# AVianEco/Softspoken

Hardware: AMD Instinct MI355X
Metric: audio-seconds processed/sec (whole node), 16 kHz mono (higher is better)
Workload: dtype f16x2

## Files before the change

softspoken_amd/build.py:

```python
from __future__ import annotations

import os
import subprocess
import sys

HERE = os.path.dirname(os.path.abspath(__file__))
CSRC = os.path.join(HERE, "csrc")
OBJ = os.path.join(CSRC, "_obj")
LIB = os.path.join(HERE, "libsoftspoken_hip.so")
DEV_LIB = os.path.join(HERE, "libsoftspoken_hip_dev.so")
SOURCES = ["conv2.hip", "conv2_ups.hip", "conv4.hip", "conv4_ups.hip", "conv1s.hip", "conv9s.hip", "conv9a.hip", "frontend.hip", "heads.hip", "weights.hip", "engine.hip", "host.hip", "abi.hip", "stream.hip", "separate.hip"]
HEADERS = [os.path.join(CSRC, h) for h in ("kernels.h", "engine.h", "dsp.h", "mfma_util.h", "conv4_forms.h", "stream16.h", "net.h", "bands.h")] + [os.path.join(os.path.dirname(HERE), "include", "softspoken.h")]
FLAGS = ["-O3", "--offload-arch=gfx950", "-fPIC", "-std=c++17", "-Wno-unused-value"]
EXTRA_FLAGS = {"frontend.hip": ["-fno-slp-vectorize"], "conv4.hip": ["-fno-slp-vectorize"], "conv4_ups.hip": ["-fno-slp-vectorize"],
               "conv1s.hip": ["-fno-slp-vectorize"], "conv9s.hip": ["-fno-slp-vectorize"], "conv9a.hip": ["-fno-slp-vectorize"]}
DEV_SOURCES = ("conv2.hip", "conv2_ups.hip", "conv4.hip", "conv4_ups.hip", "conv1s.hip", "frontend.hip", "engine.hip", "weights.hip", "abi.hip", "separate.hip")
JITTER_LIB = DEV_LIB


def _hipcc():
    for cand in (os.environ.get("HIPCC"), "/opt/rocm/bin/hipcc"):
        if cand and os.path.exists(cand):
            return cand
    return "hipcc"


def _stale(target, deps):
    if not os.path.exists(target):
        return True
    t = os.path.getmtime(target)
    return any(os.path.getmtime(d) > t for d in deps)


def build(force: bool = False, verbose: bool = True, dev: bool = False, jitter: bool = False) -> str:
    dev = dev or jitter
    os.makedirs(OBJ, exist_ok=True)
    hipcc = _hipcc()
    objs, procs = [], []
# ... 28 lines not shown
```

softspoken_amd/csrc/engine.h:

```cpp
#pragma once
#include "../../include/softspoken.h"
#include "kernels.h"
#include "net.h"

#include <map>
#include <string>
#include <vector>

namespace ss {

inline size_t pcm_bytes_per_sample(int format) {
    switch (format) {
        case SS_PCM_U8: case SS_PCM_S8: return 1;
        case SS_PCM_S16: case SS_PCM_S16BE: return 2;
        case SS_PCM_S24: case SS_PCM_S24BE: return 3;
        case SS_PCM_F64: case SS_PCM_F64BE: return 8;
        default: return 4;
    }
}

int fail(ss_ctx* c, int code, const std::string& msg);
const char* thread_error();

#define HIPCHK(c, expr)                                                                                   \
// ... 7 lines not shown
static_assert(sizeof(BlobEntry) == 152, "blob entry layout");
struct Blob {
    std::map<std::string, BlobEntry> e;
    const char* base = nullptr;
    size_t size = 0;
    bool has(const std::string& k) const { return e.count(k) != 0; }
    const float* f32(const std::string& k, size_t count, std::string& err) const;
};
bool parse_blob(const void* p, size_t n, Blob& b, std::string& err);

enum Precision { kFp32 = 0, kBf16 = 1, kF16x2 = 2 };

struct ConvPlan {
    std::string name;
    void* d_w2 = nullptr; float* d_bias2 = nullptr; float* d_res_bias = nullptr; float* d_rank1 = nullptr;
    void* d_w3 = nullptr; void* d_proj = nullptr; float* d_bias3 = nullptr;
    void* d_w_ups = nullptr;
    bool s1_range_proven = false;
    void* d_w_s1 = nullptr;
    void* d_w_s16 = nullptr;
    void* d_proj_s16 = nullptr;
    void* d_w_a16 = nullptr; void* d_w_ups16 = nullptr;
    void* d_w_upsr = nullptr;
    void* d_w_ups32 = nullptr;
    int ups32_nt = 1;
    int Cout = 0, NT = 1, C0 = 0, C1 = 0, R0 = 0, R1 = 0, H = 0, W = 0;
};

struct BlockPlan { ConvPlan A, B; };

struct FileRec {
    int64_t off = 0;
    int64_t n = 0;
    int64_t n_padded = 0;
    double duration = 0;
    int64_t W = 0, win_base = 0;
    int64_t bin_off = 0; int n_bins = 0;
};

struct StreamSet;
struct SepState;

struct SepPlan {
    int N = 0, hop = 0;
    int64_t W = 0, n_bins = 0, windows_run = 0;
    std::vector<ss_separation_range> ranges;
// ... 183 lines not shown
```

softspoken_amd/csrc/engine.hip:

```cpp
#include "engine.h"

#include <algorithm>
#include <chrono>
#include <cmath>
#include <cstdio>
#include <cstdlib>
#include <cstring>

namespace ss {

static thread_local std::string g_err;

int fail(ss_ctx* c, int code, const std::string& msg) {
    g_err = msg;
    if (c) c->err = msg;
    return code;
}
const char* thread_error() { return g_err.c_str(); }

double now_ms() { return std::chrono::duration<double, std::milli>(std::chrono::steady_clock::now().time_since_epoch()).count(); }

static int stat_id(ss_ctx* c, const std::string& name) {
    for (size_t i = 0; i < c->stats.size(); ++i) if (c->stats[i].name == name) return (int)i;
    KStat k; k.name = name; c->stats.push_back(k);
// ... 45 lines not shown
    c->dbg_n = 0; c->dbg_ws = 0; c->dbg_written = 0;
    for (Workspace& w : c->ws) free_ws(w);
}

static hipError_t ws_malloc(ss_ctx* c, void** p, size_t bytes) {
    if (c->fail_alloc_after >= 0 && c->fail_alloc_after-- == 0) { *p = nullptr; return hipErrorOutOfMemory; }
    return hipMalloc(p, bytes);
}

static hipError_t alloc_ws(ss_ctx* c, int n, hipStream_t stream, Workspace& w, std::string& what) {
    const size_t es = c->prec == kFp32 ? 4 : 2;
    size_t total = 0;
    std::vector<size_t> offs;
    for (const ActInfo& t : kActs) {
        offs.push_back(total + kActHeader);
        total += kActHeader + (((size_t)n * t.H * t.W * t.C * es + 255) & ~(size_t)255);
    }
    const int planes = c->prec == kF16x2 ? 2 : 1;
    const size_t feat_b = (size_t)n * 128 * 256 * 4, flat_b = (size_t)n * 64 * 4 * 256 * 4;
    hipError_t e = ws_malloc(c, &w.arena, total * planes);
    if (e != hipSuccess) { what = "activation workspace (" + std::to_string(total * planes >> 20) + " MiB)"; free_ws(w); return e; }
    if ((e = ws_malloc(c, (void**)&w.feat, feat_b)) != hipSuccess || (e = ws_malloc(c, (void**)&w.flat, flat_b)) != hipSuccess) {
        what = "activation workspace"; free_ws(w); return e;
    }
    for (int pl = 0; pl < planes; ++pl)
        for (size_t off : offs) {
            e = hipMemsetAsync((char*)w.arena + pl * total + off - kActHeader, 0, kActHeader, stream);
            if (e != hipSuccess) { what = "hipMemsetAsync"; free_ws(w); return e; }
        }
    const bool planar = c->prec == kF16x2 && dev_env("SOFTSPOKEN_LAYOUT", kActChunkPlanar ? 1 : 0) != 0;
    for (int i = 0; i < kActCount; ++i) {
        const ActInfo& t = kActs[i];
        w.t[i].p = (char*)w.arena + offs[i];
        if (c->prec != kFp32) w.t[i].s = act_stride(t.H, t.W, t.C, planar && !t.frag_order);
    }
    w.lo_delta = planes == 2 ? (int64_t)total : 0;
    w.bytes = (int64_t)(total * planes + feat_b + flat_b);
    w.chunk = n;
    return hipSuccess;
}

int ensure_workspace(ss_ctx* c, int n) {
    if (n <= c->ws[0].chunk) return SS_OK;
    HIPCHK(c, hipStreamSynchronize(c->stream));
    if (c->lane_stream) HIPCHK(c, hipStreamSynchronize(c->lane_stream));
    free_workspace(c);
// ... 59 lines not shown

template <typename LaunchFn>
static int conv_launch(ss_ctx* c, hipStream_t stream, const char* variant, const std::string& layer, ConvArgs& a, double flops, double bytes,
                       double issued, bool stamped, LaunchFn&& launch) {
    StageStamps stamps;
    if (stamped) if (int rc = stamps.begin(c, stream, layer, a)) return rc;
    {
        ScopedLaunch sl(c, stream, std::string(variant) + "/" + layer, flops, bytes, issued);
        HIPCHK(c, launch(a));
    }
    return stamps.end(c, stream, layer, a.N);
}

enum Form {
    kNoForm,
    kConv2,
    kConv4,
    kConv4UpsPlain,
    kConv4UpsRing,
    kConv2Ups,
    kConv1Stream16,
    kConv1Stream32,
    kConv9aStream,
    kConv9Stream
};
struct Launch { Form form = kNoForm; ConvArgs a{}; };
struct BlockRun { bool proj = false; Launch A, B, B2; };

static int prec4(const ss_ctx* c) { return c->prec == kF16x2 ? 2 : 1; }
static int ups32_mtw(const ConvPlan& p) { return dev_env("SOFTSPOKEN_UPS32_MTW", 2) == 2 && p.ups32_nt < 3 ? 2 : 1; }

static void fill_args(const ss_ctx* c, const Workspace& ws, int bi, int n, bool with_spec, BlockRun& r) {
    const Block& k = kBlocks[bi];
    const BlockPlan& p = c->convs[bi];
    auto T = [&](Act t) { return t == kNoAct ? ActTensor() : ws.t[t]; };
    const ActTensor x0 = T(k.x0), x1 = T(k.x1), h = T(k.first_in_loader ? kNoAct : k.h), rr = T(k.r), y = T(k.y), pool = T(k.pool);
    ConvArgs& a = r.A.a; ConvArgs& b = r.B.a;
    a = b = ConvArgs{};
    a.N = b.N = n; a.H = b.H = k.H; a.W = b.W = k.W; a.Cout = b.Cout = k.cout; a.relu = b.relu = 1; a.store_out = b.store_out = 1;
    a.lo_delta = b.lo_delta = ws.lo_delta; a.range_flag = b.range_flag = c->d_range_flag; a.dbg = b.dbg = base_dbg();
    a.src0 = x0.p; a.s_src0 = x0.s; a.src1 = x1.p; a.s_src1 = x1.s; a.C0 = k.c0; a.C1 = k.c1; a.out = h.p; a.s_out = h.s; a.bias = p.A.d_bias2;
    b.src0 = h.p; b.s_src0 = h.s; b.C0 = k.cout; b.out = y.p; b.s_out = y.s; b.pool_out = pool.p; b.s_pool = pool.s; b.wpk = p.B.d_w2;
    if (r.proj) {
        a.wpk = p.A.d_w3; a.plain = 1;
        b.bias = p.B.d_bias3; b.proj_w = p.B.d_proj; b.xp0 = x0.p; b.s_xp0 = x0.s; b.xp1 = x1.p; b.s_xp1 = x1.s; b.C0x = k.c0; b.C1x = k.c1;
    } else {
        a.wpk = p.A.d_w2; a.res_out = rr.p; a.res_bias = p.A.d_res_bias;
        b.bias = p.B.d_bias2; b.res_in = rr.p; b.rank1_w = p.B.d_rank1;
    }
    if (k.first_in_loader) { b.first_w = c->d_first_w; b.first_b = c->d_first_b; b.rank1_src = ws.feat; }
    if (k.flat_in_b) { b.flat_w = r.proj ? nullptr : c->d_flat_frag; b.flat_w4 = c->d_flat_frag4; b.flat_part = ws.flat; b.store_out = with_spec ? 1 : 0; }
}

static bool choose_tile(const ss_ctx* c, const ConvPlan& p, Launch& l) {
    if (c->prec != kFp32 && dev_env("SOFTSPOKEN_CONV4", 1) && conv_v4_supports(l.a, p.NT, c->num_cus, prec4(c))) l.form = kConv4;
    else if (c->prec != kF16x2) l.form = kConv2;
    return l.form != kNoForm;
}

static bool choose_A(const ss_ctx* c, const ConvPlan& p, Launch& l) {
    Launch u = l;
    if (c->prec == kF16x2 && p.d_w_upsr) {
        u.form = kConv4UpsRing; u.a.wpk = p.d_w_upsr;
        if (conv_upsr_supports(u.a, c->num_cus)) { l = u; return true; }
    }
    if (c->prec == kFp32 && p.d_w_ups32 && l.a.src1) {
        u.form = kConv2Ups; u.a.wpk = p.d_w_ups32;
        if (conv_ups32_supports(u.a, p.ups32_nt, ups32_mtw(p), c->num_cus)) { l = u; return true; }
    }
    return choose_tile(c, p, l);
}

static bool choose_B(const ss_ctx* c, const Block& k, const ConvPlan& p, BlockRun& r) {
    if (c->prec == kF16x2 && k.first_in_loader && p.d_w_s16 && dev_env("SOFTSPOKEN_C1S", 1)) {
        Launch s = r.B;
        s.form = dev_env("SOFTSPOKEN_C1S_FORM", 16) == 32 && p.d_w_s1 ? kConv1Stream32 : kConv1Stream16;
        s.a.wpk = s.form == kConv1Stream16 ? p.d_w_s16 : p.d_w_s1;
        s.a.relu = 1 | (dev_env("SOFTSPOKEN_C1S_ABLATE", 0) << 4);
        s.a.plain = p.s1_range_proven && dev_env("SOFTSPOKEN_C1S_TRACK", 0) == 0;
        if (conv1_stream_supports(s.a)) {
            if (dev_env("SOFTSPOKEN_C1S", 1) == 2) { r.B2 = r.B; if (!choose_tile(c, p, r.B2)) return false; }
            r.B = s;
            return true;
        }
// ... 32 lines not shown
        fill_args(c, ws, bi, n, with_spec, r);
        if (choose_proj(c, k, p, r)) return true;
        r = BlockRun();
    }
    fill_args(c, ws, bi, n, with_spec, r);
    if (!k.first_in_loader && !choose_A(c, p.A, r.A)) return false;
    return choose_B(c, k, p.B, r);
}

static double launch_macs(const Block& k, bool isA, bool proj, int n) {
    const double px = (double)n * k.H * k.W, cin = k.c0 + k.c1;
    if (isA) return px * k.cout * (9.0 * cin + (proj ? 0.0 : cin));
    return px * k.cout * (9.0 * k.cout + (proj ? cin : 0.0) + (k.first_in_loader ? 1 : 0)) + (k.first_in_loader ? px * 32 * 9 : 0.0) +
           (k.flat_in_b ? px * 32 * 4 : 0.0);
}
static double launch_bytes(const Block& k, bool isA, bool proj, int n, double es, bool store_y) {
    const double px = (double)n * k.H * k.W, x = k.c0 + k.c1 / 4.0;
    if (isA) return px * es * (x + k.cout + (proj ? 0 : k.cout));
    return px * es * ((k.first_in_loader ? 4.0 / es : k.cout) + (proj ? x : k.r != kNoAct ? k.cout : 0) + (store_y ? k.cout : 0) + (k.pool != kNoAct ? k.cout / 4.0 : 0));
}
static double launch_issued(const Block& k, Form f, int n) {
    const double px = (double)n * k.H * k.W;
    switch (f) {
        case kConv4UpsRing: case kConv2Ups: return px * k.cout * (9.0 * k.c0 + 4.0 * k.c1 + (k.c0 + k.c1));
        case kConv4UpsPlain: return px * k.cout * (9.0 * k.c0 + 4.0 * k.c1);
        case kConv9aStream: return conv9a_stream_issued_macs(n);
        case kConv9Stream: return conv9_stream_issued_macs(n);
        default: return -1.0;
    }
}
static int flat_groups_of(const ss_ctx* c, Form f) {
    return f == kConv9Stream ? conv9_stream_flat_groups(dev_env("SOFTSPOKEN_C9S_ROWS", 32)) : f == kConv4 ? conv_v4_flat_groups() : conv_v2_flat_groups(c->bf16);
}

static int launch_form(ss_ctx* c, hipStream_t stream, const ConvPlan& p, Launch& l, double flops, double bytes, double issued) {
    const int cus = c->num_cus;
    auto go = [&](const char* variant, auto&& launch) { return conv_launch(c, stream, variant, p.name, l.a, flops, bytes, issued, l.form != kConv4UpsPlain, launch); };
    switch (l.form) {
        case kConv2: return go(conv_v2_variant(l.a, c->bf16, p.NT, cus), [&](ConvArgs& x) { return launch_conv3x3_v2(x, c->bf16, p.NT, cus, stream); });
        case kConv4: return go(conv_v4_variant(l.a, p.NT, cus, prec4(c)), [&](ConvArgs& x) { return launch_conv3x3_v4(x, p.NT, cus, prec4(c), stream); });
        case kConv4UpsPlain: return go(conv_ups_variant(), [&](ConvArgs& x) { return launch_conv3x3_ups(x, cus, stream); });
        case kConv4UpsRing: return go(conv_upsr_variant(), [&](ConvArgs& x) { return launch_conv3x3_upsr(x, cus, stream); });
        case kConv2Ups: return go(conv_ups32_variant(p.ups32_nt, ups32_mtw(p)), [&](ConvArgs& x) { return launch_conv3x3_ups32(x, p.ups32_nt, ups32_mtw(p), cus, stream); });
        case kConv1Stream16: case kConv1Stream32: {
            const int form = l.form == kConv1Stream16 ? 16 : 32;
            return go(conv1_stream_variant(l.a, form), [&](ConvArgs& x) { return launch_conv1_stream(x, form, dev_env("SOFTSPOKEN_C1S_ROWS", 32), cus, stream); });
        }
        case kConv9aStream:
            return go(conv9a_stream_variant(), [&](ConvArgs& x) { return launch_conv9a_stream(x, dev_env("SOFTSPOKEN_C9A_ROWS", 32), dev_env("SOFTSPOKEN_C9A_GRID", 0), cus, stream); });
        case kConv9Stream:
            return go(conv9_stream_variant(), [&](ConvArgs& x) { return launch_conv9_stream(x, dev_env("SOFTSPOKEN_C9S_ROWS", 32), dev_env("SOFTSPOKEN_C9S_GRID", 0), cus, stream); });
        case kNoForm: break;
    }
    return fail(c, SS_ERR_STATE, "no kernel form chosen for " + p.name);
}

static int run_block(ss_ctx* c, Workspace& ws, hipStream_t stream, int bi, int n, bool with_spec) {
    const Block& k = kBlocks[bi];
    const BlockPlan& p = c->convs[bi];
    BlockRun r;
    if (!choose_block(c, ws, bi, n, with_spec, r))
        return fail(c, SS_ERR_STATE, "f16x2: no kernel form for " + (k.first_in_loader || r.A.form != kNoForm ? p.B.name : p.A.name));
    const bool hasA = r.A.form != kNoForm, store_y = r.B.a.store_out != 0;
    for (Act t : {hasA ? k.h : kNoAct, hasA && !r.proj ? k.r : kNoAct, store_y ? k.y : kNoAct, k.pool})
        if (t != kNoAct) c->dbg_written |= (uint64_t)1 << t;
    const double es = c->prec == kBf16 ? 2 : 4;
    for (Launch* l : {&r.A, &r.B, &r.B2}) {
        if (l->form == kNoForm) continue;
        const bool isA = l == &r.A;
        if (int rc = launch_form(c, stream, isA ? p.A : p.B, *l, 2.0 * launch_macs(k, isA, r.proj, n), launch_bytes(k, isA, r.proj, n, es, store_y),
                                 launch_issued(k, l->form, n)))
            return rc;
// ... 354 lines not shown
```

softspoken_amd/csrc/kernels.h:

```cpp
#pragma once
#include <hip/hip_runtime.h>
#include <stdint.h>
#include <atomic>
#include <cstdlib>

namespace ss {

#ifdef SS_DEVBUILD
static inline int dev_env(const char* name, int dflt) { const char* v = getenv(name); return v ? atoi(v) : dflt; }
#else
static constexpr int dev_env(const char*, int dflt) { return dflt; }
#endif

inline hipError_t allow_full_lds(const void* kernel, std::atomic<uint64_t>& done) {
    int dev = 0;
    hipError_t e = hipGetDevice(&dev);
    if (e != hipSuccess) return e;
    const uint64_t bit = 1ull << (dev & 63);
    if (done.load(std::memory_order_acquire) & bit) return hipSuccess;
    e = hipFuncSetAttribute(kernel, hipFuncAttributeMaxDynamicSharedMemorySize, 160 * 1024);
    if (e == hipSuccess) done.fetch_or(bit, std::memory_order_release);
    return e;
}

// ... 102 lines not shown
hipError_t launch_conv3x3_ups32(const ConvArgs& a, int NT, int MTW, int num_cus, hipStream_t s);

bool conv1_stream_supports(const ConvArgs& a);
const char* conv1_stream_variant(const ConvArgs& a, int form);
size_t conv1_stream_weight_bytes();
hipError_t launch_conv1_stream(const ConvArgs& a, int form, int rows_per_unit, int num_cus, hipStream_t s);

bool conv9_stream_supports(const ConvArgs& a);
const char* conv9_stream_variant();
size_t conv9_stream_proj_bytes();
size_t conv9_stream_flat_bytes();
bool conv9_stream_rows_ok(int rows_per_unit);
int conv9_stream_flat_groups(int rows_per_unit);
double conv9_stream_issued_macs(int N);
hipError_t launch_conv9_stream(const ConvArgs& a, int rows_per_unit, int grid_override, int num_cus, hipStream_t s);

bool conv9a_stream_supports(const ConvArgs& a);
const char* conv9a_stream_variant();
size_t conv9a_stream_ups_bytes();
bool conv9a_stream_rows_ok(int rows_per_unit);
double conv9a_stream_issued_macs(int N);
hipError_t launch_conv9a_stream(const ConvArgs& a, int rows_per_unit, int grid_override, int num_cus, hipStream_t s);

struct Head1dWeights { float w1[4][4][3], b1[4], w2[4][4][3], wr[4][4], b2r[4], wo[4], bo, fscale; };
hipError_t launch_mask_head_parts(const float* parts, int n_parts, const float* flat_bias, const Head1dWeights& hw, float* logits,
                                  int N, hipStream_t s);
hipError_t launch_spec_tail(const void* x, int64_t lo_delta, const float* w , const float* bias, float* spec, int N, int prec,
                            hipStream_t s);

static constexpr int kMelLo = 10, kMelHi = 32, kMelPitch = 43;
struct FrontendTables {
    const float4* pretw;
    const float2* w2048;
    const int* mel_start;
    const int* mel_count;
    const int* mel_off;
    const float* mel_w;
    int mel_nw;
    const float* mel_wp;
    int dbg;
    const float2* win2;
    const float2* twt;
    const float2* wkt;
    const float* mel_wq;
    const int* mel_p0;
};
// ... 54 lines not shown
```

softspoken_amd/csrc/weights.hip:

```cpp
#include "engine.h"

#include <algorithm>
#include <cmath>
#include <cstring>

namespace ss {

const float* Blob::f32(const std::string& k, size_t count, std::string& err) const {
    auto it = e.find(k);
    if (it == e.end()) { err = "weights blob: missing tensor '" + k + "'"; return nullptr; }
    if (it->second.dtype != 0 || it->second.nbytes != count * 4) {
        err = "weights blob: tensor '" + k + "' has wrong dtype/size"; return nullptr;
    }
    return (const float*)(base + it->second.offset);
}

bool parse_blob(const void* p, size_t n, Blob& b, std::string& err) {
    if (n < 16 || memcmp(p, "SSWBLOB1", 8) != 0) { err = "weights blob: bad magic"; return false; }
    uint32_t cnt; memcpy(&cnt, (const char*)p + 8, 4);
    if (16 + (size_t)cnt * sizeof(BlobEntry) > n) { err = "weights blob: truncated table"; return false; }
    b.base = (const char*)p; b.size = n;
    for (uint32_t i = 0; i < cnt; ++i) {
        BlobEntry en; memcpy(&en, (const char*)p + 16 + (size_t)i * sizeof(BlobEntry), sizeof(BlobEntry));
        en.name[95] = 0;
// ... 207 lines not shown
}

static void pack_ups_stream16(const Folded& w3, int c0, std::vector<char>& out, bool& range_ok) {
    out.assign((size_t)2 * 2 * 4 * 2 * 2 * 1024, 0);
    static const int lo_of[2][2] = {{0, 1}, {0, 2}}, hi_of[2][2] = {{0, 2}, {1, 2}};
    for (int a = 0; a < 2; ++a)
        for (int ty = 0; ty < 2; ++ty)
            for (int f = 0; f < 4; ++f)
                for (int u = 0; u < 2; ++u)
                    for (int l = 0; l < 64; ++l)
                        for (int j = 0; j < 8; ++j) {
                            const int b = f >> 1, tx = f & 1, i = l & 15, co = 8 * (i >> 2) + 4 * u + (i & 3), ci = c0 + 8 * (l >> 4) + j;
                            double sum = 0.0;
                            for (int dy = lo_of[a][ty]; dy <= hi_of[a][ty]; ++dy)
                                for (int dx = lo_of[b][tx]; dx <= hi_of[b][tx]; ++dx) sum += (double)w3.w[((size_t)co * w3.cin + ci) * 9 + dy * 3 + dx];
                            const float v = (float)sum;
                            const uint16_t hi = f2h(v), lo = f2h(v - h2f(hi));
                            if ((hi & 0x7c00u) == 0x7c00u) range_ok = false;
                            const size_t off = ((size_t)((((a * 2 + ty) * 4 + f) * 2 + u) * 2) * 64 + l) * 16 + (size_t)j * 2;
                            memcpy(&out[off], &hi, 2); memcpy(&out[off + 1024], &lo, 2);
                        }
}

static void pack_conv_split_upsr(const Folded& w3, const Folded& wr, int c0, int c1, std::vector<char>& out, bool& range_ok) {
    const size_t ent_r = (size_t)10 * 2048, ent_rh = ent_r + 256, ent_u = (size_t)17 * 2048;
    const int nreg = c0 / 32, nups = c1 / 32, ngroups = w3.cout / 32;
    const size_t group = (size_t)nreg * (ent_rh + ent_r) + (size_t)nups * 2 * ent_u;
    out.assign((size_t)ngroups * group, 0);
    auto put = [&](size_t off_hi, size_t off_lo, float v) {
        const uint16_t hi = f2h(v), lo = f2h(v - h2f(hi));
        if ((hi & 0x7c00u) == 0x7c00u) range_ok = false;
        memcpy(&out[off_hi], &hi, 2); memcpy(&out[off_lo], &lo, 2);
    };
    static const int lo_of[2][2] = {{0, 1}, {0, 2}}, hi_of[2][2] = {{0, 2}, {1, 2}};
    for (int g = 0; g < ngroups; ++g) {
        const size_t gb = (size_t)g * group;
        for (int ci = 0; ci < nreg; ++ci) {
            const size_t eh = gb + (size_t)ci * (ent_rh + ent_r), el = eh + ent_rh;
            for (int t = 0; t < 10; ++t)
                for (int s = 0; s < 2; ++s)
                    for (int l = 0; l < 64; ++l)
                        for (int e = 0; e < 8; ++e) {
                            const int co = g * 32 + (l & 31), k = ci * 32 + s * 16 + (l >> 5) * 8 + e;
                            const float v = t < 9 ? w3.w[((size_t)co * w3.cin + k) * 9 + t] : wr.w[(size_t)co * wr.cin + k];
                            const size_t off = (size_t)t * 2048 + ((size_t)s * 64 + l) * 16 + (size_t)e * 2;
                            put(eh + off, el + off, v);
// ... 270 lines not shown
                bh[co] = q; worst = std::max(worst, q);
            }
            for (int co = 0; co < cout; ++co) {
                double q = std::fabs((double)b2r[co]) + std::fabs((double)fr.w[co]) * fmax;
                for (int ci = 0; ci < cout; ++ci)
                    for (int t = 0; t < 9; ++t) q += std::fabs((double)f2.w[((size_t)co * cout + ci) * 9 + t]) * bh[ci];
                worst = std::max(worst, q);
            }
            B.s1_range_proven = std::isfinite(worst) && worst < 60000.0;
        }
        out.B = B;
        return SS_OK;
    }
    const int NTA = (c->prec == kF16x2 && NT == 3) ? 1 : NT;
    ConvPlan A; A.name = name + ".A"; A.Cout = cout; A.NT = NTA; A.C0 = cin0; A.C1 = cin1; A.H = H; A.W = W;
    if ((rc = dev_upload(c, &A.d_bias2, f1.b.data(), cout * 4))) return rc;
    if (c->prec == kF16x2) pack_conv_split(f1, &fr, NTA, pk, c->split_range_ok); else pack_conv_v2(f1, &fr, c->bf16, NT, pk);
    if ((rc = dev_upload(c, (char**)&A.d_w2, pk.data(), pk.size()))) return rc;
    if ((rc = dev_upload(c, &A.d_res_bias, fr.b.data(), cout * 4))) return rc;
    if (c->prec == kF16x2 && NTA == 1 && cin0 >= 64 && cin0 % 32 == 0 && cin1 % 32 == 0 && (cin1 >= 32 || dev_env("SOFTSPOKEN_UPSR", 1) >= 2)) {
        pack_conv_split_upsr(f1, fr, cin0, cin1, pk, c->split_range_ok);
        if (pk.size() != conv_upsr_weight_bytes(cin0, cin1, cout)) return fail(c, SS_ERR_STATE, "pack_conv_split_upsr: size");
        if ((rc = dev_upload(c, (char**)&A.d_w_upsr, pk.data(), pk.size()))) return rc;
    }
    if (c->prec == kFp32 && cin1 >= 16 && cin0 % 16 == 0 && cin1 % 16 == 0 && cout % 32 == 0 && H % 16 == 0 && dev_env("SOFTSPOKEN_UPS32", 1)) {
        A.ups32_nt = dev_env("SOFTSPOKEN_UPS32_NT", 1);
        if (A.ups32_nt < 1 || A.ups32_nt > 3 || (cout / 32) % A.ups32_nt) A.ups32_nt = 1;
        pack_conv_v2_ups(f1, fr, cin0, cin1, A.ups32_nt, pk);
        if (pk.size() != conv_ups32_weight_bytes(cin0, cin1, cout)) return fail(c, SS_ERR_STATE, "pack_conv_v2_ups: size");
        if ((rc = dev_upload(c, (char**)&A.d_w_ups32, pk.data(), pk.size()))) return rc;
    }
    if (c->bf16) {
        pack_conv_v2(f1, nullptr, true, NT, pk);
        if ((rc = dev_upload(c, (char**)&A.d_w3, pk.data(), pk.size()))) return rc;
    }
    if (c->prec == kF16x2) {
        pack_conv_split(f1, nullptr, NTA, pk, c->split_range_ok);
        if ((rc = dev_upload(c, (char**)&A.d_w3, pk.data(), pk.size()))) return rc;
        if (cin1 >= 32 && cin0 >= 32 && cout == 32) {
            pack_conv_split_ups(f1, cin0, cin1, pk, c->split_range_ok);
            if (pk.size() != conv_ups_weight_bytes(cin0, cin1)) return fail(c, SS_ERR_STATE, "pack_conv_split_ups: size");
            if ((rc = dev_upload(c, (char**)&A.d_w_ups, pk.data(), pk.size()))) return rc;
            if (cin0 == 32 && cin1 == 32 && H == 128 && W == 256) {
                pack_conv_stream16(f1, pk, c->split_range_ok);
                if (pk.size() != conv1_stream_weight_bytes()) return fail(c, SS_ERR_STATE, "pack_conv_stream16: size");
                if ((rc = dev_upload(c, (char**)&A.d_w_a16, pk.data(), pk.size()))) return rc;
// ... 155 lines not shown
```

Measured before the change: 35390.

## Add streaming fused skip+upsample conv kernel for 64x128 decoder A-conv

Adds a new streaming kernel for the f16x2 decoder conv that fuses the 3x3 skip conv, the folded 2x upsample conv and the 1x1 residual projection. Each wave walks rows of a 32-wide strip, holding a register ring of weights staged through LDS and software-pipelining row loads against MFMA groups. The kernel is chosen by default for the 64x128, 64+64->32 layer ahead of the existing ups-ring kernel. It targets redundant activation reads and per-tile launch overhead. The cost is a specialised, shape-locked kernel with heavy register pressure. A debug workspace-poison option is also added.

```diff
diff --git a/softspoken_amd/build.py b/softspoken_amd/build.py
--- a/softspoken_amd/build.py
+++ b/softspoken_amd/build.py
@@ -9,11 +9,11 @@
 OBJ = os.path.join(CSRC, "_obj")
 LIB = os.path.join(HERE, "libsoftspoken_hip.so")
 DEV_LIB = os.path.join(HERE, "libsoftspoken_hip_dev.so")
-SOURCES = ["conv2.hip", "conv2_ups.hip", "conv4.hip", "conv4_ups.hip", "conv1s.hip", "conv9s.hip", "conv9a.hip", "frontend.hip", "heads.hip", "weights.hip", "engine.hip", "host.hip", "abi.hip", "stream.hip", "separate.hip"]
+SOURCES = ["conv2.hip", "conv2_ups.hip", "conv4.hip", "conv4_ups.hip", "conv1s.hip", "conv9s.hip", "conv9a.hip", "conv8a.hip", "frontend.hip", "heads.hip", "weights.hip", "engine.hip", "host.hip", "abi.hip", "stream.hip", "separate.hip"]
 HEADERS = [os.path.join(CSRC, h) for h in ("kernels.h", "engine.h", "dsp.h", "mfma_util.h", "conv4_forms.h", "stream16.h", "net.h", "bands.h")] + [os.path.join(os.path.dirname(HERE), "include", "softspoken.h")]
 FLAGS = ["-O3", "--offload-arch=gfx950", "-fPIC", "-std=c++17", "-Wno-unused-value"]
 EXTRA_FLAGS = {"frontend.hip": ["-fno-slp-vectorize"], "conv4.hip": ["-fno-slp-vectorize"], "conv4_ups.hip": ["-fno-slp-vectorize"],
-               "conv1s.hip": ["-fno-slp-vectorize"], "conv9s.hip": ["-fno-slp-vectorize"], "conv9a.hip": ["-fno-slp-vectorize"]}
+               "conv1s.hip": ["-fno-slp-vectorize"], "conv9s.hip": ["-fno-slp-vectorize"], "conv9a.hip": ["-fno-slp-vectorize"], "conv8a.hip": ["-fno-slp-vectorize"]}
 DEV_SOURCES = ("conv2.hip", "conv2_ups.hip", "conv4.hip", "conv4_ups.hip", "conv1s.hip", "frontend.hip", "engine.hip", "weights.hip", "abi.hip", "separate.hip")
 JITTER_LIB = DEV_LIB
 
diff --git a/softspoken_amd/csrc/conv8a.hip b/softspoken_amd/csrc/conv8a.hip
--- /dev/null
+++ b/softspoken_amd/csrc/conv8a.hip
@@ -0,0 +1,301 @@
+#include "kernels.h"
+#include "stream16.h"
+#include <algorithm>
+#include <type_traits>
+#include <utility>
+
+namespace ss {
+
+namespace {
+
+constexpr int kH8 = 64, kW8 = 128, kStrips8 = 4;
+constexpr uint32_t kRow2 = kW8 * 64, kRow7 = (kW8 / 2) * 64;
+constexpr uint32_t kChunk2 = kH8 * kRow2, kChunk7 = (kH8 / 2) * kRow7;
+constexpr int kSkip8 = 2 * 9 * 2048;
+constexpr int kUps8 = 2 * 4 * 4 * 2048;
+constexpr int kProj8 = 4 * 2048;
+constexpr int kTile8 = kSkip8 + kUps8 + kProj8;
+constexpr uint32_t kRWin = (kH8 / 2) * (kW8 / 16) * 2048;
+
+struct G8 { int kind, off, k, a, b, flags; };
+template <int DY, int RF, int PROJ, int C7FIRST>
+struct Seq8 {
+    G8 g[40];
+    int n;
+    constexpr void c2_groups() {
+        for (int k = 0; k < 2; ++k)
+            for (int dxi = 0; dxi < 3; ++dxi) {
+                bool first = true;
+                for (int dyi = 0; dyi < 3; ++dyi)
+                    if ((DY >> dyi) & 1) { g[n++] = G8{0, ((k * 9 + dyi * 3 + dxi) * 2) * 1024, k, dyi, dxi, (first ? 1 : 0) | (first && !RF && k == 1 && dxi == 0 ? 4 : 0)}; first = false; }
+                if (dxi == 1 && PROJ) g[n++] = G8{1, kSkip8 + kUps8 + k * 2048, k, 0, 0, 0};
+            }
+        if (RF && !C7FIRST) g[n - 1].flags |= 2;
+    }
+    constexpr void c7_groups() {
+        if (PROJ) g[n++] = G8{3, kSkip8 + kUps8 + 2 * 2048, 0, 0, 0, 0};
+        for (int k = 0; k < 2; ++k)
+            for (int pt = 0; pt < 2; ++pt) {
+                bool first = true;
+                for (int rf = 0; rf < 4; ++rf)
+                    if ((RF >> rf) & 1) { g[n++] = G8{2, kSkip8 + (((k * 4 + rf) * 4 + pt) * 2) * 1024, k, rf, pt, (first ? 1 : 0) | (first && k == 1 && pt == 1 ? 4 : 0)}; first = false; }
+            }
+    }
+    constexpr Seq8() : g{}, n(0) {
+        if (RF && C7FIRST) c7_groups();
+        c2_groups();
+        if (RF && !C7FIRST) c7_groups();
+    }
+};
+template <int DY, int RF, int PROJ, int STOREH, int EDGE, int INIT, int C7OFF, int LAST>
+struct SD8 {
+    static constexpr int dy = DY, rf = RF, proj = PROJ, storeh = STOREH, edge = EDGE, init = INIT, c7off = C7OFF, last = LAST;
+    static constexpr int c7first = C7OFF != 0;
+    static constexpr Seq8<DY, RF, PROJ, c7first> seq{};
+};
+using StepPro = SD8<1, 8, 0, 0, 1, 1, -1, 0>;
+using StepEvenFirst = SD8<3, 14, 1, 0, 0, 3, 0, 0>;
+using StepOdd = SD8<7, 0, 1, 1, 0, 0, 0, 0>;
+using StepEven = SD8<7, 15, 1, 1, 0, 3, 0, 0>;
+using StepEvenLast = SD8<7, 7, 1, 1, 0, 1, 0, 0>;
+using StepOddLast = SD8<6, 0, 1, 1, 0, 0, 0, 0>;
+using StepEpi = SD8<4, 1, 0, 1, 1, 0, 0, 1>;
+static_assert(StepPro::seq.n == 10 && StepEvenFirst::seq.n == 27 && StepOdd::seq.n == 20 && StepEven::seq.n == 37 && StepEvenLast::seq.n == 33 &&
+              StepOddLast::seq.n == 14 && StepEpi::seq.n == 10, "groups per step");
+static_assert((2 + 10) % 3 == 0 && (0 + 27) % 3 == 0 && (0 + 20) % 3 == 2 && (2 + 37) % 3 == 0 && (2 + 33) % 3 == 2 && (2 + 14) % 3 == 1 &&
+              (1 + 10) % 3 == 2, "ring phases");
+
+template <int... I, typename F>
+__device__ __forceinline__ void static_for_(std::integer_sequence<int, I...>, F&& f) { (f(std::integral_constant<int, I>{}), ...); }
+template <int N, typename F>
+__device__ __forceinline__ void static_for(F&& f) { static_for_(std::make_integer_sequence<int, N>{}, f); }
+
+struct C8Row7 { u32x4 f[2]; u32x4 h[2]; };
+struct C8Ring { u32x4 w[3][4]; };
+
+}
+
+__global__ __launch_bounds__(64 * kS1Waves) __attribute__((amdgpu_waves_per_eu(2, 2)))
+void conv3x3_upsr_stream16_kernel(ConvArgs a, int rows_per_unit, int total_units) {
+    extern __shared__ __attribute__((aligned(16))) char smem[];
+    const int tid = threadIdx.x, lane = tid & 63, wave = __builtin_amdgcn_readfirstlane(tid >> 6);
+    const int g = lane >> 4, c = lane & 15;
+    const int u = __builtin_amdgcn_readfirstlane(((int)blockIdx.x >> 3) & 1);
+    const int pair = __builtin_amdgcn_readfirstlane(((int)blockIdx.x & 7) + 8 * ((int)blockIdx.x >> 4)), npairs = (int)gridDim.x >> 1;
+    {
+        const char* src = (const char*)a.wpk + (size_t)u * kTile8;
+        for (int p = tid; p < kTile8 / 16; p += 64 * kS1Waves) *(u32x4*)(smem + p * 16) = *(const u32x4*)(src + (size_t)p * 16);
+    }
+    const f32x4 bias = *(const f32x4*)(a.bias + 16 * u + 4 * g), rbias = *(const f32x4*)(a.res_bias + 16 * u + 4 * g);
+    __syncthreads();
+
+    const char* fl = smem + lane * 16;
+    auto rsrc_of = [](const void* p, uint32_t bytes) { return __builtin_amdgcn_make_buffer_rsrc(const_cast<void*>(p), 0, (int)bytes, 0x00020000); };
+    auto ld16 = [](__amdgpu_buffer_rsrc_t rs, uint32_t vo, int so) { return __builtin_bit_cast(u32x4, __builtin_amdgcn_raw_buffer_load_b128(rs, (int)vo, so, 0)); };
+    const uint32_t px2 = a.s_src0.pix, ch2 = a.s_src0.chunk, px7 = a.s_src1.pix, ch7 = a.s_src1.chunk;
+    const uint32_t vpix = (uint32_t)(2 * c) * px2 + (uint32_t)g * 16u, vpix7 = (uint32_t)c * px7 + (uint32_t)g * 16u;
+    const uint32_t vout = (uint32_t)(2 * c) * 64u + 32u * (uint32_t)u + 8u * (uint32_t)g;
+    const uint32_t vr = (uint32_t)(c >> 3) * 2048u + (uint32_t)(32 * (g & 1) + 4 * (c & 7)) * 32u + 16u * (uint32_t)(g >> 1);
+    const int bands = kH8 / rows_per_unit;
+    const int64_t lo = a.lo_delta;
+    uint32_t ovf = 0;
+    C8Ring ring;
+    uint32_t far_ = 65536u;
+    asm volatile("" : "+v"(far_));
+    const char* fl_hi = fl + far_;
+    auto rd_group = [&](int slot, const G8 gd) {
+        const char* p = gd.off + (gd.kind >= 2 ? 4096 + 1024 : 1024) < 65536 ? fl + gd.off : fl_hi + (gd.off - 65536);
+        ring.w[slot][0] = *(const u32x4*)(p); ring.w[slot][1] = *(const u32x4*)(p + 1024);
+        if (gd.kind >= 2) {
+            const int d = gd.kind == 2 ? 4096 : 2048;
+            ring.w[slot][2] = *(const u32x4*)(p + d); ring.w[slot][3] = *(const u32x4*)(p + d + 1024);
+        }
+    };
+    { constexpr G8 g0 = StepPro::seq.g[0], g1 = StepPro::seq.g[1]; rd_group(2, g0); rd_group(0, g1); }
+
+    for (int unit = pair * kS1Waves + wave; unit < total_units; unit += npairs * kS1Waves) {
+        const int s = unit % kStrips8, b = (unit / kStrips8) % bands, n = unit / (kStrips8 * bands);
+        const int x0 = 32 * s, y0 = b * rows_per_unit, ylast = y0 + rows_per_unit - 1;
+        const uint32_t hpix = (uint32_t)(c < 8 ? max(x0 - 1, 0) : min(x0 + 32, kW8 - 1)) * px2 + (uint32_t)g * 16u;
+        const uint32_t hpix7 = (uint32_t)(c < 8 ? max(x0 / 2 - 1, 0) : min(x0 / 2 + 16, kW8 / 2 - 1)) * px7 + (uint32_t)g * 16u;
+        const uint32_t hkeep = (c < 8 ? s > 0 : s < kStrips8 - 1) ? 0xffffffffu : 0u;
+        const char* c2w = (const char*)a.src0 + (size_t)n * 2 * kChunk2;
+        const char* c7w = (const char*)a.src1 + (size_t)n * 2 * kChunk7;
+        const __amdgpu_buffer_rsrc_t rs2[2] = {rsrc_of(c2w, 2 * kChunk2), rsrc_of(c2w + lo, 2 * kChunk2)};
+        const __amdgpu_buffer_rsrc_t rs7[2] = {rsrc_of(c7w, 2 * kChunk7), rsrc_of(c7w + lo, 2 * kChunk7)};
+        char* ow = (char*)a.out + (size_t)n * kChunk2;
+        const __amdgpu_buffer_rsrc_t rso[2] = {rsrc_of(ow, kChunk2), rsrc_of(ow + lo, kChunk2)};
+        const __amdgpu_buffer_rsrc_t rsr = rsrc_of((char*)a.res_out + (size_t)u * lo + (size_t)n * kRWin, kRWin);
+
+        auto load_chunk = [&](S16RowH& H, int k, int r) {
+            const int so = (min(max(r, 0), kH8 - 1) * kW8 + x0) * (int)px2 + k * (int)ch2;
+#pragma unroll
+            for (int pq = 0; pq < 2; ++pq) {
+                H.f[0][pq] = ld16(rs2[pq], vpix, so);
+                H.f[1][pq] = ld16(rs2[pq], vpix, so + (int)px2);
+                H.h[pq] = ld16(rs2[pq], hpix, so - x0 * (int)px2);
+            }
+        };
+        auto load_row7 = [&](C8Row7 (&K)[2], int r7) {
+            const int so = (min(max(r7, 0), kH8 / 2 - 1) * (kW8 / 2) + x0 / 2) * (int)px7;
+#pragma unroll
+            for (int k = 0; k < 2; ++k)
+#pragma unroll
+                for (int pq = 0; pq < 2; ++pq) {
+                    K[k].f[pq] = ld16(rs7[pq], vpix7, so + k * (int)ch7);
+                    K[k].h[pq] = ld16(rs7[pq], hpix7, so - (x0 / 2) * (int)px7 + k * (int)ch7);
+                }
+        };
+        S16RowH Hrow[2][2];
+        C8Row7 K[2];
+        f32x4 A[4][2];
+        f32x4 R[2], RU, RUa, RUb;
+        uint32_t ovt = 0;
+
+        auto step = [&](auto cur, auto next, auto rho4_c, auto ph_c, int rho) {
+            using Cur = decltype(cur); using Next = decltype(next);
+            constexpr int RHO4 = decltype(rho4_c)::value, PH = decltype(ph_c)::value, N = Cur::seq.n;
+            S16RowH (&Hc)[2] = Hrow[RHO4 & 1];
+            const int Y = (rho + Cur::c7off) >> 1;
+            S16RowH (&Hn)[2] = Hrow[(RHO4 & 1) ^ 1];
+            if constexpr (!Cur::last && (Cur::rf == 0 || Cur::c7first)) load_chunk(Hn[0], 0, rho + 1);
+            if constexpr (Cur::rf != 0 && !Cur::c7first) load_row7(K, Y);
+            auto mask_row7 = [&]() {
+                const uint32_t rk = !Cur::edge || (unsigned)Y < (unsigned)(kH8 / 2) ? 0xffffffffu : 0u;
+#pragma unroll
+                for (int k = 0; k < 2; ++k)
+#pragma unroll
+                    for (int pq = 0; pq < 2; ++pq)
+#pragma unroll
+                        for (int e = 0; e < 4; ++e) {
+                            if constexpr (Cur::edge) K[k].f[pq][e] &= rk;
+                            K[k].h[pq][e] &= hkeep & rk;
+                        }
+            };
+            if constexpr (Cur::c7first) mask_row7();
+            {
+                const uint32_t rk = !Cur::edge || (unsigned)rho < (unsigned)kH8 ? 0xffffffffu : 0u;
+#pragma unroll
+                for (int k = 0; k < 2; ++k)
+#pragma unroll
+                    for (int pq = 0; pq < 2; ++pq)
+#pragma unroll
+                        for (int e = 0; e < 4; ++e) {
+                            if constexpr (Cur::edge) { Hc[k].f[0][pq][e] &= rk; Hc[k].f[1][pq][e] &= rk; }
+                            Hc[k].h[pq][e] &= hkeep & rk;
+                        }
+            }
+            if constexpr (Cur::init & 1) { A[(RHO4 + 1) & 3][0] = bias; A[(RHO4 + 1) & 3][1] = bias; }
+            if constexpr (Cur::init & 2) { A[(RHO4 + 2) & 3][0] = bias; A[(RHO4 + 2) & 3][1] = bias; }
+            u32x4 B[2][2];
+            static_for<N>([&](auto I) {
+                constexpr int i = decltype(I)::value, slot = (PH + i) % 3;
+                constexpr G8 gd = Cur::seq.g[i];
+                if constexpr (i + 2 < N) { constexpr G8 gn = Cur::seq.g[i + 2]; rd_group((PH + i + 2) % 3, gn); }
+                else { constexpr G8 gn = Next::seq.g[i + 2 - N]; rd_group((PH + i + 2) % 3, gn); }
+                if constexpr ((gd.flags & 4) != 0 && !Cur::last) load_chunk(Hn[1], 1, rho + 1);
+                if constexpr (gd.kind == 0 && (gd.flags & 1)) {
+#pragma unroll
+                    for (int pq = 0; pq < 2; ++pq) { B[0][pq] = s16_operand(Hc[gd.k], gd.b - 1, 0, pq); B[1][pq] = s16_operand(Hc[gd.k], gd.b - 1, 1, pq); }
+                }
+                if constexpr (gd.kind == 2 && (gd.flags & 1)) {
+#pragma unroll
+                    for (int pq = 0; pq < 2; ++pq) {
+                        B[0][pq] = gd.b == 0 ? s16_shr1_halo(K[gd.k].f[pq], K[gd.k].h[pq]) : K[gd.k].f[pq];
+                        B[1][pq] = gd.b == 0 ? K[gd.k].f[pq] : s16_shl1_halo(K[gd.k].f[pq], K[gd.k].h[pq]);
+                    }
+                }
+                if constexpr (gd.kind == 3) { RUa = f32x4{0.f, 0.f, 0.f, 0.f}; RUb = RUa; }
+                if constexpr (gd.kind == 1 && gd.k == 0) { R[0] = rbias; R[1] = rbias; }
+                __builtin_amdgcn_sched_barrier(0);
+#pragma unroll
+                for (int pr = 0; pr < 3; ++pr) {
+                    const int pq = pr == 0 ? 1 : 0, wq = pr == 1 ? 1 : 0;
+                    if constexpr (gd.kind == 0) {
+                        f32x4 (&P)[2] = A[(RHO4 + 1 - gd.a) & 3];
+                        P[0] = s16_mfma(ring.w[slot][wq], B[0][pq], P[0]);
+                        P[1] = s16_mfma(ring.w[slot][wq], B[1][pq], P[1]);
+                    } else if constexpr (gd.kind == 1) {
+                        R[0] = s16_mfma(ring.w[slot][wq], Hc[gd.k].f[0][pq], R[0]);
+                        R[1] = s16_mfma(ring.w[slot][wq], Hc[gd.k].f[1][pq], R[1]);
+                    } else if constexpr (gd.kind == 2) {
+                        f32x4 (&P)[2] = A[(RHO4 + Cur::c7off - 1 + gd.a) & 3];
+                        P[0] = s16_mfma(ring.w[slot][wq], B[0][pq], P[0]);
+                        P[1] = s16_mfma(ring.w[slot][2 + wq], B[1][pq], P[1]);
+                    } else {
+                        RUa = s16_mfma(ring.w[slot][wq], K[0].f[pq], RUa);
+                        RUb = s16_mfma(ring.w[slot][2 + wq], K[1].f[pq], RUb);
+                    }
+                }
+                __builtin_amdgcn_sched_barrier(0);
+                if constexpr ((gd.flags & 2) != 0) {
+                    if constexpr (!Cur::last) load_chunk(Hn[0], 0, rho + 1);
+                    mask_row7();
+                }
+            });
+            if constexpr (Cur::storeh) {
+                const int so = (rho - 1) * (int)kRow2 + x0 * 64;
+#pragma unroll
+                for (int t = 0; t < 2; ++t) {
+                    const f32x4 v = A[(RHO4 + 3) & 3][t];
+                    const float v0 = relu_i(v[0]), v1 = relu_i(v[1]), v2 = relu_i(v[2]), v3 = relu_i(v[3]);
+                    const uint32_t kh0 = pack_f16(v0, v1), kh1 = pack_f16(v2, v3);
+                    const uint32_t kl0 = split_lo(kh0, v0, v1), kl1 = split_lo(kh1, v2, v3);
+                    ovt = pk_max_u16(pk_max_u16(ovt, kh0), kh1);
+                    __builtin_amdgcn_raw_buffer_store_b64(u32x2{kh0, kh1}, rso[0], (int)vout, so + 64 * t, 0);
+                    __builtin_amdgcn_raw_buffer_store_b64(u32x2{kl0, kl1}, rso[1], (int)vout, so + 64 * t, 0);
+                }
+            }
+            if constexpr (Cur::proj) {
+                if constexpr (Cur::rf != 0) RU = RUa + RUb;
+                R[0] += RU; R[1] += RU;
+                const int so = ((rho >> 1) * (kW8 / 16) + 2 * s) * 2048 + (rho & 1) * 64;
+                __builtin_amdgcn_raw_buffer_store_b128(__builtin_bit_cast(u32x4, R[0]), rsr, (int)vr, so, 0);
+                __builtin_amdgcn_raw_buffer_store_b128(__builtin_bit_cast(u32x4, R[1]), rsr, (int)vr, so + 32, 0);
+            }
+        };
+
+        load_chunk(Hrow[1][0], 0, y0 - 1); load_chunk(Hrow[1][1], 1, y0 - 1); load_row7(K, (y0 >> 1) - 1);
+        const std::integral_constant<int, 0> i0; const std::integral_constant<int, 1> i1; const std::integral_constant<int, 2> i2; const std::integral_constant<int, 3> i3;
+        step(StepPro{}, StepEvenFirst{}, i3, i2, y0 - 1);
+        step(StepEvenFirst{}, StepOdd{}, i0, i0, y0);
+        for (int y = y0 + 1; y + 2 < ylast; y += 4) {
+            step(StepOdd{}, StepEven{}, i1, i0, y);
+            step(StepEven{}, StepOdd{}, i2, i2, y + 1);
+            step(StepOdd{}, StepEven{}, i3, i0, y + 2);
+            step(StepEven{}, StepOdd{}, i0, i2, y + 3);
+        }
+        step(StepOdd{}, StepEvenLast{}, i1, i0, ylast - 2);
+        step(StepEvenLast{}, StepOddLast{}, i2, i2, ylast - 1);
+        step(StepOddLast{}, StepEpi{}, i3, i2, ylast);
+        step(StepEpi{}, StepPro{}, i0, i1, ylast + 1);
+        ovf = pk_max_u16(ovf, ovt);
+    }
+    if (((ovf & 0x7fff7fffu) + 0x04000400u) & 0x80008000u) atomicOr(a.range_flag, 1);
+}
+
+bool conv8a_stream_supports(const ConvArgs& a) {
+    return !a.plain && a.H == kH8 && a.W == kW8 && a.Cout == 32 && a.C0 == 64 && a.C1 == 64 && a.src0 && a.src1 && a.wpk && a.bias && a.res_bias &&
+           a.out && a.res_out && !a.pool_out && !a.res_in && a.relu && a.lo_delta > 0 && a.range_flag && a.N > 0 &&
+           ((a.s_src0.pix == 64u && a.s_src0.chunk == kChunk2) || (a.s_src0.pix == 128u && a.s_src0.chunk == 64u)) &&
+           ((a.s_src1.pix == 64u && a.s_src1.chunk == kChunk7) || (a.s_src1.pix == 128u && a.s_src1.chunk == 64u)) && a.s_out.pix == 64u;
+}
+const char* conv8a_stream_variant() { return "conv3x3_upsr_stream16_kernel"; }
+size_t conv8a_stream_weight_bytes() { return 2 * (size_t)kTile8; }
+bool conv8a_stream_rows_ok(int rows_per_unit) { return rows_per_unit >= 4 && rows_per_unit % 4 == 0 && kH8 % rows_per_unit == 0 && rows_per_unit <= kMaxRows; }
+
+hipError_t launch_conv8a_stream(const ConvArgs& a, int rows_per_unit, int grid_override, int num_cus, hipStream_t s) {
+    if (!conv8a_stream_supports(a) || !conv8a_stream_rows_ok(rows_per_unit)) return hipErrorInvalidValue;
+    const int64_t total = (int64_t)a.N * (kH8 / rows_per_unit) * kStrips8;
+    if (total >= (int64_t)1 << 30) return hipErrorInvalidValue;
+    const int cus = num_cus > 0 ? num_cus : 256;
+    int64_t pairs = std::min<int64_t>(cus / 2, (total + kS1Waves - 1) / kS1Waves);
+    if (grid_override > 0) pairs = std::min<int64_t>(pairs, grid_override);
+    const int grid = (int)std::max<int64_t>(1, pairs / 8) * 16;
+    static std::atomic<uint64_t> attr_done{0};
+    if (hipError_t e = allow_full_lds((const void*)conv3x3_upsr_stream16_kernel, attr_done)) return e;
+    hipLaunchKernelGGL(conv3x3_upsr_stream16_kernel, dim3(grid), dim3(64 * kS1Waves), (size_t)kTile8, s, a, rows_per_unit, (int)total);
+    return hipGetLastError();
+}
+
+}
diff --git a/softspoken_amd/csrc/engine.h b/softspoken_amd/csrc/engine.h
--- a/softspoken_amd/csrc/engine.h
+++ b/softspoken_amd/csrc/engine.h
@@ -53,6 +53,7 @@
     void* d_proj_s16 = nullptr;
     void* d_w_a16 = nullptr; void* d_w_ups16 = nullptr;
     void* d_w_upsr = nullptr;
+    void* d_w_c8s = nullptr;
     void* d_w_ups32 = nullptr;
     int ups32_nt = 1;
     int Cout = 0, NT = 1, C0 = 0, C1 = 0, R0 = 0, R1 = 0, H = 0, W = 0;
diff --git a/softspoken_amd/csrc/engine.hip b/softspoken_amd/csrc/engine.hip
--- a/softspoken_amd/csrc/engine.hip
+++ b/softspoken_amd/csrc/engine.hip
@@ -91,6 +91,10 @@
     if (e != hipSuccess) { what = "activation workspace (" + std::to_string(total * planes >> 20) + " MiB)"; free_ws(w); return e; }
     if ((e = ws_malloc(c, (void**)&w.feat, feat_b)) != hipSuccess || (e = ws_malloc(c, (void**)&w.flat, flat_b)) != hipSuccess) {
         what = "activation workspace"; free_ws(w); return e;
+    }
+    if (dev_env("SOFTSPOKEN_WS_POISON", 0)) {
+        e = hipMemsetAsync(w.arena, 0xff, total * planes, stream);
+        if (e != hipSuccess) { what = "hipMemsetAsync"; free_ws(w); return e; }
     }
     for (int pl = 0; pl < planes; ++pl)
         for (size_t off : offs) {
@@ -196,6 +200,7 @@
     kConv1Stream16,
     kConv1Stream32,
     kConv9aStream,
+    kConv8aStream,
     kConv9Stream
 };
 struct Launch { Form form = kNoForm; ConvArgs a{}; };
@@ -234,6 +239,11 @@
 
 static bool choose_A(const ss_ctx* c, const ConvPlan& p, Launch& l) {
     Launch u = l;
+    if (c->prec == kF16x2 && p.d_w_c8s && dev_env("SOFTSPOKEN_C8S", 1) && dev_env("SOFTSPOKEN_UPSR", 1)) {
+        u.form = kConv8aStream; u.a.wpk = p.d_w_c8s;
+        if (conv8a_stream_supports(u.a) && conv8a_stream_rows_ok(dev_env("SOFTSPOKEN_C8S_ROWS", 32))) { l = u; return true; }
+        u = l;
+    }
     if (c->prec == kF16x2 && p.d_w_upsr) {
         u.form = kConv4UpsRing; u.a.wpk = p.d_w_upsr;
         if (conv_upsr_supports(u.a, c->num_cus)) { l = u; return true; }
@@ -312,7 +322,7 @@
 static double launch_issued(const Block& k, Form f, int n) {
     const double px = (double)n * k.H * k.W;
     switch (f) {
-        case kConv4UpsRing: case kConv2Ups: return px * k.cout * (9.0 * k.c0 + 4.0 * k.c1 + (k.c0 + k.c1));
+        case kConv4UpsRing: case kConv2Ups: case kConv8aStream: return px * k.cout * (9.0 * k.c0 + 4.0 * k.c1 + (k.c0 + k.c1));
         case kConv4UpsPlain: return px * k.cout * (9.0 * k.c0 + 4.0 * k.c1);
         case kConv9aStream: return conv9a_stream_issued_macs(n);
         case kConv9Stream: return conv9_stream_issued_macs(n);
@@ -325,7 +335,9 @@
 
 static int launch_form(ss_ctx* c, hipStream_t stream, const ConvPlan& p, Launch& l, double flops, double bytes, double issued) {
     const int cus = c->num_cus;
-    auto go = [&](const char* variant, auto&& launch) { return conv_launch(c, stream, variant, p.name, l.a, flops, bytes, issued, l.form != kConv4UpsPlain, launch); };
+    auto go = [&](const char* variant, auto&& launch) {
+        return conv_launch(c, stream, variant, p.name, l.a, flops, bytes, issued, l.form != kConv4UpsPlain && l.form != kConv8aStream, launch);
+    };
     switch (l.form) {
         case kConv2: return go(conv_v2_variant(l.a, c->bf16, p.NT, cus), [&](ConvArgs& x) { return launch_conv3x3_v2(x, c->bf16, p.NT, cus, stream); });
         case kConv4: return go(conv_v4_variant(l.a, p.NT, cus, prec4(c)), [&](ConvArgs& x) { return launch_conv3x3_v4(x, p.NT, cus, prec4(c), stream); });
@@ -338,6 +350,8 @@
         }
         case kConv9aStream:
             return go(conv9a_stream_variant(), [&](ConvArgs& x) { return launch_conv9a_stream(x, dev_env("SOFTSPOKEN_C9A_ROWS", 32), dev_env("SOFTSPOKEN_C9A_GRID", 0), cus, stream); });
+        case kConv8aStream:
+            return go(conv_upsr_variant(), [&](ConvArgs& x) { return launch_conv8a_stream(x, dev_env("SOFTSPOKEN_C8S_ROWS", 32), dev_env("SOFTSPOKEN_C8S_GRID", 0), cus, stream); });
         case kConv9Stream:
             return go(conv9_stream_variant(), [&](ConvArgs& x) { return launch_conv9_stream(x, dev_env("SOFTSPOKEN_C9S_ROWS", 32), dev_env("SOFTSPOKEN_C9S_GRID", 0), cus, stream); });
         case kNoForm: break;
diff --git a/softspoken_amd/csrc/kernels.h b/softspoken_amd/csrc/kernels.h
--- a/softspoken_amd/csrc/kernels.h
+++ b/softspoken_amd/csrc/kernels.h
@@ -148,6 +148,12 @@
 double conv9a_stream_issued_macs(int N);
 hipError_t launch_conv9a_stream(const ConvArgs& a, int rows_per_unit, int grid_override, int num_cus, hipStream_t s);
 
+bool conv8a_stream_supports(const ConvArgs& a);
+const char* conv8a_stream_variant();
+size_t conv8a_stream_weight_bytes();
+bool conv8a_stream_rows_ok(int rows_per_unit);
+hipError_t launch_conv8a_stream(const ConvArgs& a, int rows_per_unit, int grid_override, int num_cus, hipStream_t s);
+
 struct Head1dWeights { float w1[4][4][3], b1[4], w2[4][4][3], wr[4][4], b2r[4], wo[4], bo, fscale; };
 hipError_t launch_mask_head_parts(const float* parts, int n_parts, const float* flat_bias, const Head1dWeights& hw, float* logits,
                                   int N, hipStream_t s);
diff --git a/softspoken_amd/csrc/weights.hip b/softspoken_amd/csrc/weights.hip
--- a/softspoken_amd/csrc/weights.hip
+++ b/softspoken_amd/csrc/weights.hip
@@ -253,6 +253,38 @@
                         }
 }
 
+static void pack_conv8a_stream(const Folded& w3, const Folded& wr, int c0, std::vector<char>& out, bool& range_ok) {
+    const size_t skip = (size_t)2 * 9 * 2048, ups = (size_t)2 * 16 * 2048, proj = (size_t)4 * 2048, tile = skip + ups + proj;
+    out.assign(2 * tile, 0);
+    auto put = [&](size_t off_hi, float v) {
+        const uint16_t hi = f2h(v), lo = f2h(v - h2f(hi));
+        if ((hi & 0x7c00u) == 0x7c00u) range_ok = false;
+        memcpy(&out[off_hi], &hi, 2); memcpy(&out[off_hi + 1024], &lo, 2);
+    };
+    static const int lo_of[2][2] = {{0, 1}, {0, 2}}, hi_of[2][2] = {{0, 2}, {1, 2}};
+    static const int rf_a[4] = {1, 0, 1, 0}, rf_ty[4] = {1, 1, 0, 0};
+    for (int u = 0; u < 2; ++u)
+        for (int l = 0; l < 64; ++l)
+            for (int j = 0; j < 8; ++j) {
+                const int co = 16 * u + (l & 15), kk = 8 * (l >> 4) + j;
+                const size_t at = (size_t)u * tile + (size_t)l * 16 + (size_t)j * 2;
+                for (int k = 0; k < 2; ++k) {
+                    const int ci = 32 * k + kk, cu = c0 + 32 * k + kk;
+                    for (int t = 0; t < 9; ++t) put(at + (size_t)(k * 9 + t) * 2048, w3.w[((size_t)co * w3.cin + ci) * 9 + t]);
+                    for (int rf = 0; rf < 4; ++rf)
+                        for (int f = 0; f < 4; ++f) {
+                            const int a = rf_a[rf], ty = rf_ty[rf], b = f >> 1, tx = f & 1;
+                            double sum = 0.0;
+                            for (int dy = lo_of[a][ty]; dy <= hi_of[a][ty]; ++dy)
+                                for (int dx = lo_of[b][tx]; dx <= hi_of[b][tx]; ++dx) sum += (double)w3.w[((size_t)co * w3.cin + cu) * 9 + dy * 3 + dx];
+                            put(at + skip + (size_t)((k * 4 + rf) * 4 + f) * 2048, (float)sum);
+                        }
+                    put(at + skip + ups + (size_t)k * 2048, wr.w[(size_t)co * wr.cin + ci]);
+                    put(at + skip + ups + (size_t)(2 + k) * 2048, wr.w[(size_t)co * wr.cin + cu]);
+                }
+            }
+}
+
 static void pack_conv_split_upsr(const Folded& w3, const Folded& wr, int c0, int c1, std::vector<char>& out, bool& range_ok) {
     const size_t ent_r = (size_t)10 * 2048, ent_rh = ent_r + 256, ent_u = (size_t)17 * 2048;
     const int nreg = c0 / 32, nups = c1 / 32, ngroups = w3.cout / 32;
@@ -569,6 +601,11 @@
         pack_conv_split_upsr(f1, fr, cin0, cin1, pk, c->split_range_ok);
         if (pk.size() != conv_upsr_weight_bytes(cin0, cin1, cout)) return fail(c, SS_ERR_STATE, "pack_conv_split_upsr: size");
         if ((rc = dev_upload(c, (char**)&A.d_w_upsr, pk.data(), pk.size()))) return rc;
+        if (cin0 == 64 && cin1 == 64 && cout == 32 && H == 64 && W == 128) {
+            pack_conv8a_stream(f1, fr, cin0, pk, c->split_range_ok);
+            if (pk.size() != conv8a_stream_weight_bytes()) return fail(c, SS_ERR_STATE, "pack_conv8a_stream: size");
+            if ((rc = dev_upload(c, (char**)&A.d_w_c8s, pk.data(), pk.size()))) return rc;
+        }
     }
     if (c->prec == kFp32 && cin1 >= 16 && cin0 % 16 == 0 && cin1 % 16 == 0 && cout % 32 == 0 && H % 16 == 0 && dev_env("SOFTSPOKEN_UPS32", 1)) {
         A.ups32_nt = dev_env("SOFTSPOKEN_UPS32_NT", 1);
```

After: 35740 (median of 6 runs). About the same (+1.0%).
